# CentreForHydrology/WDPM

Hardware: AMD Instinct MI355X
Metric: cell-updates/sec on Add module, 16384x16384 DEM (higher is better)
Workload: dtype f64

## Files before the change

### wdpm_amd/csrc/wdpm_capi.hip

```cpp
#include <hip/hip_runtime.h>

#include <time.h>

#include <cmath>
#include <cstdarg>
#include <cstdio>
#include <cstdlib>
#include <cstring>
#include <atomic>
#include <vector>

#include "wdpm_ctx.h"

constexpr int kSparseChunkRows = 96;

static thread_local char g_err[512] = "";

int wdpm_fail(const char *fmt, ...) {
  va_list ap;
  va_start(ap, fmt);
  vsnprintf(g_err, sizeof g_err, fmt, ap);
  va_end(ap);
  return 1;
}
// ... 250 lines not shown
  x->w_negative = false;
  x->w_odd = true;
  x->launches = 0;
  x->ms = 0.0;
  x->steady_launches = 0;
  x->steady_ms = 0.0;
  x->timing = false; x->xch_count = 0; x->xch_ms = 0.0;
  x->comm = nullptr;
  x->leak = false;
  x->d_dem = x->d_w[0] = x->d_w[1] = x->d_w[2] = nullptr;
  x->old = 2;
  for (int i = 0; i < 3; i++) { x->d_zero[i] = nullptr; x->zero_valid[i] = false; }
  x->tile_cap = x->tile_nstrips = x->tile_H = x->tile_nchunks = 0;
  x->d_active = nullptr; x->h_active = nullptr;
  x->tiles_launched = 0; x->sparse = false; x->stat_tiles = x->stat_active = 0;
  x->wide_tri_ok = false; x->blocks_unprobed = 0;
  memset(&x->bal, 0, sizeof x->bal);
  { const char *e = getenv("WDPM_TILES"); x->tiles_mode = e ? atoi(e) : 1; }
  x->flush_pending = false;
  x->d_md = nullptr; x->md_hint = x->md_valid = false; x->md_lo = x->md_hi = 0;
  x->drain_owed = false;
  x->flush_thres = -__builtin_inf();
  x->d_scal = nullptr; x->d_bits = nullptr; x->h_pin = nullptr; x->d_stat = nullptr; x->h_iter2_err = x->d_iter2_err = nullptr;
  x->d_dem32 = nullptr; x->code = DemCode{nullptr, 0.0, 1.0, 1.0, 0, nullptr, nullptr, 0}; x->dem32_encodable = false; x->dem_bounded = false;
  x->d_dem16 = nullptr; x->d_gbase = nullptr; x->dem16_encodable = false; x->dem16_wanted = true;
  x->graph_mode = -1; x->graph_launches = 0;
  x->d_sum_approx = nullptr; x->d_sum_i = nullptr; x->d_sum_k = nullptr; x->d_sum_flag = nullptr;
  x->own_stream = true;
  x->side = nullptr; x->ev_fork = nullptr; x->ev_join = nullptr; x->pending_join = false; x->ev_copy[0] = x->ev_copy[1] = nullptr;
  const size_t bytes = x->cells * sizeof(double);
  hipError_t e = hipStreamCreateWithFlags(&x->stream, hipStreamNonBlocking);
  int prio_least = 0, prio_greatest = 0;
  if (e == hipSuccess) e = hipDeviceGetStreamPriorityRange(&prio_least, &prio_greatest);
  if (e == hipSuccess) e = hipStreamCreateWithPriority(&x->side, hipStreamNonBlocking, prio_least);
  if (e == hipSuccess) e = hipEventCreateWithFlags(&x->ev_fork, hipEventDisableTiming);
  if (e == hipSuccess) e = hipEventCreateWithFlags(&x->ev_join, hipEventDisableTiming);
  if (e == hipSuccess) e = guarded_malloc(x, (void **)&x->d_dem, bytes + 192 * sizeof(double));
  if (e == hipSuccess) e = guarded_malloc(x, (void **)&x->d_w[0], bytes + 192 * sizeof(double));
  if (e == hipSuccess) e = guarded_malloc(x, (void **)&x->d_w[1], bytes + 192 * sizeof(double));
  if (e == hipSuccess) e = guarded_malloc(x, (void **)&x->d_w[2], bytes + 192 * sizeof(double));
  if (e == hipSuccess) e = guarded_malloc(x, (void **)&x->d_dem32, x->cells * sizeof(int) + 64);
  if (e == hipSuccess) e = guarded_malloc(x, (void **)&x->d_dem16, x->cells * sizeof(unsigned short) + 64);
  if (e == hipSuccess) e = guarded_malloc(x, (void **)&x->d_gbase, (size_t)x->g.rows * ((x->g.ncp + kDemGroup - 1) / kDemGroup) * sizeof(int) + 64);
  if (e == hipSuccess) e = hipMalloc(&x->d_scal, 2 * sizeof(double));
  if (e == hipSuccess) e = hipMalloc(&x->d_bits, 2 * sizeof(unsigned long long));
  if (e == hipSuccess) e = hipMalloc(&x->d_md, sizeof(unsigned long long));
  if (e == hipSuccess) {
// ... 123 lines not shown
  q.flags = launch_flags(x);
  q.leave_cus = leave_cus;
  q.codes32 = x->code.q != nullptr;
  q.codes16 = x->code.h != nullptr;
  q.force_codes = x->code.force;
  q.tiles_offered = tiles != nullptr;
  q.tile_capacity = tiles && tiles->zout ? tiles->capacity : 0;
  q.wide_tri_ok = tiles && tiles->wide_tri_ok;
  q.balance_mode = balanced ? x->bal.mode : 0;
  q.balance_capacity = x->bal.capacity;
  return q;
}

static void drop_graphs(wdpm_ctx *x) {
  if (x->graphs.empty()) return;
  (void)hipStreamSynchronize(x->stream);
  for (auto &ge : x->graphs) (void)hipGraphExecDestroy(ge.exec);
  x->graphs.clear();
}

static int encode_dem(wdpm_ctx *x) {
  drop_graphs(x);
  x->dem32_encodable = false; x->dem16_encodable = false; x->dem_bounded = false; x->dem16_wanted = true;
  x->code = DemCode{nullptr, 0.0, 1.0, 1.0, 0, nullptr, nullptr, 0};
  HIP_TRY(wdpm_launch_dem_min(x->d_dem, x->cells, x->d_bits, x->stream));
  HIP_TRY(hipMemcpyAsync(x->h_pin, x->d_bits, 2 * sizeof(double), hipMemcpyDeviceToHost, x->stream));
  if (wdpm_stream_sync(x, x->stream)) return 1;
  unsigned long long key, amax;
  memcpy(&key, x->h_pin, sizeof key);
  memcpy(&amax, x->h_pin + 1, sizeof amax);
  x->dem_bounded = amax < 0x41d0000000000000ull;
  const char *env = getenv("WDPM_DEM32");
  if (env && atoi(env) == 0) return 0;
  if (key == ~0ull) return 0;
  const double vmin = wdpm_dem_key_to_double(key);
  static const double p10[7] = {1.0, 1e1, 1e2, 1e3, 1e4, 1e5, 1e6};
  for (int e = 0; e <= 6; e++) {
    const double D = p10[e], rD = 1.0 / D, k0 = rint(vmin * D);
    if (!(fabs(k0) < 4.0e15)) break;
    HIP_TRY(wdpm_launch_dem_encode(x->d_dem, x->cells, k0, D, rD, x->d_dem32, x->d_bits, x->stream));
    HIP_TRY(hipMemcpyAsync(x->h_pin, x->d_bits, sizeof(double), hipMemcpyDeviceToHost, x->stream));
    if (wdpm_stream_sync(x, x->stream)) return 1;
    unsigned long long bad;
    memcpy(&bad, x->h_pin, sizeof bad);
    if (!bad) {
      x->dem32_encodable = true;
      x->code = DemCode{x->d_dem32, k0, D, rD, (env && atoi(env) == 2) ? 1 : 0, nullptr, nullptr, 0};
      break;
    }
  }
  const char *env16 = getenv("WDPM_DEM16");
  if (x->dem32_encodable && !(env16 && atoi(env16) == 0)) {
    const int ngroups = (x->g.ncp + kDemGroup - 1) / kDemGroup;
    HIP_TRY(wdpm_launch_dem16_encode(x->d_dem32, x->g.rows, x->g.ncp, ngroups, x->d_dem16, x->d_gbase, x->d_bits, x->stream));
    HIP_TRY(hipMemcpyAsync(x->h_pin, x->d_bits, sizeof(double), hipMemcpyDeviceToHost, x->stream));
    if (wdpm_stream_sync(x, x->stream)) return 1;
    unsigned long long bad;
    memcpy(&bad, x->h_pin, sizeof bad);
    if (!bad) {
      x->dem16_encodable = true;
      x->code.h = x->d_dem16;
      x->code.gb = x->d_gbase;
      x->code.ngroups = ngroups;
    }
  }
  return 0;
}

int wdpm_upload(wdpm_ctx *x, const double *bigdem, const double *bigwater) {
  if (!bigdem || !bigwater) return fail("wdpm_upload: null array");
  if (bind(x)) return 1;
  const size_t bytes = x->cells * sizeof(double);
  if (ensure_fresh_slot(x)) return 1;
  HIP_TRY(hipMemcpyAsync(x->d_dem, bigdem, bytes, hipMemcpyHostToDevice, x->stream));
  HIP_TRY(hipMemcpyAsync(x->d_w[x->cur], bigwater, bytes, hipMemcpyHostToDevice, x->stream));
  HIP_TRY(wdpm_launch_mark_nodata(x->d_dem, x->cells, x->g.miss, x->stream));
  x->signed_zero_safe = x->w_negative = x->w_odd = false;
// ... 739 lines not shown
```

### wdpm_amd/csrc/wdpm_fused.hip

```cpp
#include "wdpm_kernels.h"
#include "wdpm_ledger.h"
#include "wdpm_stencil.h"

#include <atomic>
#include <cstring>
#include <mutex>
#include <type_traits>

namespace {


#define WDPM_INF (__builtin_inf())

__device__ __forceinline__ double lane_next(const double v) {
  int lo = __double2loint(v), hi = __double2hiint(v);
  lo = __builtin_amdgcn_update_dpp(0, lo, 0x130, 0xF, 0xF, true);
  hi = __builtin_amdgcn_update_dpp(0, hi, 0x130, 0xF, 0xF, true);
  return __hiloint2double(hi, lo);
}

__device__ __forceinline__ double lane_prev(const double v, const double keep) {
  int lo = __double2loint(v), hi = __double2hiint(v);
  lo = __builtin_amdgcn_update_dpp(__double2loint(keep), lo, 0x138, 0xF, 0xF, false);
  hi = __builtin_amdgcn_update_dpp(__double2hiint(keep), hi, 0x138, 0xF, 0xF, false);
// ... 149 lines not shown
                       D[a][2], da0, da1, D[b][2], db0, db1, D[c][2], dc0, dc1,
                       rd0, rd1, rd2, cdr[2], cdr[3], cdr[4], ds);
  W[a][0] = lane_prev(wa0, W[a][0]);  W[a][1] = lane_prev(wa1, W[a][1]);
  W[b][0] = lane_prev(wb0, W[b][0]);  W[b][1] = lane_prev(wb1, W[b][1]);
  W[c][0] = lane_prev(wc0, W[c][0]);  W[c][1] = lane_prev(wc1, W[c][1]);
}

template <int MODULE, bool SZ_SAFE, int NSTAGES = 3, int PLAIN = 0>
__device__ __forceinline__ void three_stages(double (&W)[7][3], const double (&D)[7][3], const int rbase,
                                             const int drain_row, const bool (&cdr)[5], DrainState &ds) {
  if (MODULE == 2 && drain_row >= rbase && drain_row <= rbase + 6) {
    stage_impl<MODULE, SZ_SAFE, 4, true>(W, D, rbase + 4, drain_row, cdr, ds);
    if (NSTAGES >= 2) stage_impl<MODULE, SZ_SAFE, 2, true>(W, D, rbase + 2, drain_row, cdr, ds);
    if (NSTAGES >= 3) stage_impl<MODULE, SZ_SAFE, 0, true>(W, D, rbase + 0, drain_row, cdr, ds);
  } else {
    stage_impl<MODULE, SZ_SAFE, 4, false, PLAIN>(W, D, rbase + 4, drain_row, cdr, ds);
    if (NSTAGES >= 2) stage_impl<MODULE, SZ_SAFE, 2, false, PLAIN>(W, D, rbase + 2, drain_row, cdr, ds);
    if (NSTAGES >= 3) stage_impl<MODULE, SZ_SAFE, 0, false, PLAIN>(W, D, rbase + 0, drain_row, cdr, ds);
  }
}

#ifdef WDPM_WAVE_TIMES
static __device__ unsigned long long g_wave_times[4 * 8192];
#define WDPM_RSTAMP(k) do { __builtin_amdgcn_sched_barrier(0); __builtin_amdgcn_s_waitcnt(0); rst[k] = wall_clock64(); __builtin_amdgcn_s_waitcnt(0); __builtin_amdgcn_sched_barrier(0); } while (0)
#else
#define WDPM_RSTAMP(k) do { } while (0)
#endif
#ifndef WDPM_FUSED_MIN_WAVES
#define WDPM_FUSED_MIN_WAVES 2
#endif
#ifndef WDPM_FUSED_CODES_WAVES
#define WDPM_FUSED_CODES_WAVES 2
#endif

typedef int wdpm_i3 __attribute__((ext_vector_type(3)));
struct Prefetched {
  double NW[3][3], ND[3][3];
  wdpm_i3 qi[3];
  int qh[3][3];
  int gbv[3];
};

template <int MODULE, bool SZ_SAFE, int DEM32, bool MD>
constexpr int fused_built_for() {
  return (MODULE == 2 && SZ_SAFE) ? 1 : (MODULE != 2 && DEM32 != 0 && !MD && !SZ_SAFE) ? WDPM_FUSED_CODES_WAVES : WDPM_FUSED_MIN_WAVES;
}

constexpr int kIter2Polls = 1 << 21;

template <int DEM32>
__device__ __forceinline__ void iter2_march(const double *__restrict__ win, double *__restrict__ wout, const DemCode &code, const SlabGeom &g,
                                            const int H, const int out_last, const int no_clamp, const BalanceArgs &bal, const Iter2Args &i2,
                                            const int vb, const int wave, const int lane, const int share, const int xcc_phys,
                                            double *const stage_lds) {
  extern __shared__ double i2_ring[];
  __shared__ int hand[8];
  if (threadIdx.x < 8) hand[threadIdx.x] = 0;
  __syncthreads();
  if (vb >= i2.ngroups * i2.nchunks) return;
#ifdef WDPM_WAVE_TIMES
  const unsigned long long wt0 = wall_clock64();
#endif
  const int grp = vb % i2.ngroups, chunk = vb / i2.ngroups;
  const bool producer = wave < 4;
  const int j = wave & 3;
  const int c0 = kGroupOut * grp + kStripOut * j;
  int A = H * chunk, A_next = A + H;
  if (bal.table) {
    A = bal.table[chunk * i2.ngroups + grp];
    A_next = bal.table[(chunk + 1) * i2.ngroups + grp];
    A = A < 0 ? 0 : (A > g.rows ? g.rows : A);
// ... 17 lines not shown
  int scol[3];
  bool store_any;
  {
    const int lo = j == 0 ? (grp == 0 ? 0 : kGroupHaloL) : kHaloL;
    int hi = kStripIn - 1 - (j == 3 ? kGroupHaloR : kHaloR);
    if (hi > g.ncp - 1 - c0) hi = g.ncp - 1 - c0;
    store_any = hi >= lo;
#pragma unroll
    for (int k = 0; k < 3; k++) {
      int c = lo + 64 * k + lane < hi ? lo + 64 * k + lane : hi;
      c = store_any ? c : 0;
      scol[k] = c;
      soff[k] = 8u * (unsigned)c;
    }
  }
  int dcol[3];
#pragma unroll
  for (int jj = 0; jj < 3; jj++) {
    const int cs = 3 * lane + jj;
    const bool own = cs >= (j == 0 ? 0 : kHaloL) && cs <= (j == 3 ? kStripIn - 1 : kStripIn - 1 - kHaloR);
    dcol[jj] = own ? kStripOut * j + cs : kGroupIn + jj;
  }
  const int rcol = kStripOut * j + 3 * lane;
  volatile int *const hand_v = hand;
  const int nb_lo = j > 0 ? j - 1 : 0, nb_hi = j < 3 ? j + 1 : 3;
  bool broken = false;
  auto await = [&](const int base, const int need) -> int {
    int m = 0, polls = 0;
    for (;;) {
      const int a = hand_v[base + nb_lo], b = hand_v[base + j], c = hand_v[base + nb_hi];
      m = a < b ? a : b;
      m = m < c ? m : c;
      m = __builtin_amdgcn_readfirstlane(m);
      if (m >= need || broken) break;
      if (++polls > kIter2Polls) {
        broken = true;
        if (lane == 0) *i2.err = 1u;
        break;
      }
      __builtin_amdgcn_s_sleep(2);
    }
    asm volatile("" ::: "memory");
    return m;
  };
  const size_t pitch = (size_t)g.ncp;
  char *const dump = reinterpret_cast<char *>(wout + (size_t)g.rows * pitch);
  const bool edge = (As + 3 * (nsteps + 1) > g.rows);
  double W[7][3], D[7][3];
#pragma unroll
  for (int k = 0; k < 7; k++)
#pragma unroll
    for (int jj = 0; jj < 3; jj++) { W[k][jj] = 0.0; D[k][jj] = WDPM_INF; }
  bool cdr[5];
#pragma unroll
  for (int k = 0; k < 5; k++) cdr[k] = false;
  DrainState ds;
  ds.td = 0.0;
  ds.hit = false;

  auto march = [&](auto edge_tag, auto role_tag) {
    constexpr bool EDGE = decltype(edge_tag)::value;
    constexpr bool PRODUCER = decltype(role_tag)::value;
    const int voff0 = 8 * (colb < g.ncp ? colb : g.ncp - 1);
    const int qoff0 = voff0 / 2, hoff0 = voff0 / 4, goff0 = 4 * ((voff0 / 8) / kDemGroup);
    auto prefetch = [&](Prefetched &P, const int r0) {
#pragma unroll
      for (int i = 0; i < 3; i++) {
// ... 46 lines not shown
      hand_v[4 + j] = t + 1;
    };
    double staged[3][3];
    auto read_staged = [&]() {
#pragma unroll
      for (int i = 0; i < 3; i++)
#pragma unroll
        for (int k = 0; k < 3; k++) staged[i][k] = stage_lds[i * kStripIn + scol[k]];
    };
    auto write_staged = [&](const int rb) {
#pragma unroll
      for (int i = 0; i < 3; i++) {
        const int r = rb + i;
        const bool row_ok = r >= or_lo && r <= or_hi && store_any;
        char *const orow = row_ok ? reinterpret_cast<char *>(wout + (size_t)r * pitch + c0) : dump;
#pragma unroll
        for (int k = 0; k < 3; k++) asm volatile("global_store_dwordx2 %0, %1, %2" : : "v"(soff[k]), "v"(staged[i][k]), "s"(orow) : "memory");
      }
      __builtin_amdgcn_wave_barrier();
    };

    auto step = [&](const int n, Prefetched &P, auto nstages_tag) {
      constexpr int NSTAGES = decltype(nstages_tag)::value;
      if (!PRODUCER) read_staged();
#pragma unroll
      for (int i = 0; i < 3; i++)
#pragma unroll
        for (int jj = 0; jj < 3; jj++) {
          W[4 + i][jj] = P.NW[i][jj];
          if (DEM32 == 2) D[4 + i][jj] = dem16_decode_nan(P.qh[i][jj], P.gbv[i], code.k0, code.D, code.rD);
          else D[4 + i][jj] = dem32_decode_nan(P.qi[i][jj], code.k0, code.D, code.rD);
        }
      if (EDGE) {
#pragma unroll
        for (int i = 0; i < 3; i++) {
          const bool row_ok = As + 3 * n + i < g.rows;
#pragma unroll
          for (int jj = 0; jj < 3; jj++) {
            const bool ok = row_ok & (colb + jj < g.ncp);
            W[4 + i][jj] = ok ? W[4 + i][jj] : 0.0;
            D[4 + i][jj] = ok ? D[4 + i][jj] : WDPM_INF;
          }
        }
      }
      {
        auto hi = [](const double v) { return (unsigned)__double2hiint(v); };
        auto max3 = [](const unsigned a, const unsigned b, const unsigned c) { const unsigned m = a > b ? a : b; return m > c ? m : c; };
        unsigned hm = max3(hi(W[4][0]), hi(W[4][1]), hi(W[4][2]));
        hm = max3(hm, hi(W[5][0]), hi(W[5][1]));
        hm = max3(hm, hi(W[5][2]), hi(W[6][0]));
        hm = max3(hm, hi(W[6][1]), hi(W[6][2]));
        deep = (deep & 8) | ((deep & 3) << 1) | (__ballot(hm > 0x40080000u) != 0 ? 1 : 0);
      }
      if (!PRODUCER) take(P, n + 1);
      prefetch(P, As + 3 * (n + 1));
      if (!PRODUCER) write_staged(A + 3 * (n - 1) - 4);

      const int rbase = As + 3 * n - 4;
      if (deep) three_stages<0, false, NSTAGES, 1>(W, D, rbase, g.dr, cdr, ds);
      else three_stages<0, false, NSTAGES, 1 | 2>(W, D, rbase, g.dr, cdr, ds);

      if (PRODUCER) {
        const int rr0 = 3 * n - 4 - sh;
        const int taken = await(4, n - sh / 3 - R / 3);
        if (i2.prio) {
          const int ahead = n - lag - taken;
          if (ahead <= 1) __builtin_amdgcn_s_setprio(3);
          else if (ahead >= R / 3 - 1) __builtin_amdgcn_s_setprio(0);
          else __builtin_amdgcn_s_setprio(1);
        }
#pragma unroll
        for (int i = 0; i < 3; i++) {
          double *const row = i2_ring + (size_t)(rr0 + i >= 0 ? put_slot : R) * kRingPitch;
          if (rr0 + i >= 0) put_slot = put_slot + 1 >= R ? 0 : put_slot + 1;
#pragma unroll
          for (int jj = 0; jj < 3; jj++) row[dcol[jj]] = W[i][jj];
        }
        asm volatile("" ::: "memory");
        hand_v[j] = n + 1;
      } else {
#pragma unroll
        for (int i = 0; i < 3; i++)
#pragma unroll
// ... 25 lines not shown
  };
  if (producer) {
    if (edge) march(std::true_type{}, std::true_type{});
    else march(std::false_type{}, std::true_type{});
  } else {
    if (edge) march(std::true_type{}, std::false_type{});
    else march(std::false_type{}, std::false_type{});
  }
  if (bal.acc && lane == 0) {
    const int x = chunk == i2.nchunks - 1 ? 8 : chunk == 0 ? 9 : (bal.rot ? xcc_phys : (int)(blockIdx.x & 7));
    if (!bal.rot || share == xcc_phys) {
      atomicAdd(bal.acc + x, wall_clock64() - bal_t0);
      atomicAdd(bal.acc + kBalClasses + x, 1ull);
    }
  }
#ifdef WDPM_WAVE_TIMES
  const int item = vb * 8 + wave;
  if (lane == 0 && item < 8192) {
    __builtin_amdgcn_s_waitcnt(0);
    g_wave_times[4 * item] = wt0;
    g_wave_times[4 * item + 1] = wall_clock64();
    g_wave_times[4 * item + 2] = __builtin_amdgcn_s_getreg((31 << 11) | 4) | ((unsigned long long)__builtin_amdgcn_s_getreg((3 << 11) | 20) << 32);
    g_wave_times[4 * item + 3] = ((unsigned long long)(4 * grp + j + (producer ? 0 : 0x4000)) << 48) | ((unsigned long long)(nsteps & 0xffff) << 32) | (unsigned)chunk;
  }
#endif
}

template <int MODULE, bool SZ_SAFE, int DEM32, bool FLUSH = false, bool MD = false, bool PLAIN = false>
__global__ void __launch_bounds__((fused_built_for<MODULE, SZ_SAFE, DEM32, MD>() >= 2 ? 512 : 256), (fused_built_for<MODULE, SZ_SAFE, DEM32, MD>()))
fused_iteration_kernel(const double *__restrict__ win, double *__restrict__ wout,
                       const double *__restrict__ dem, const DemCode code, const SlabGeom g, const int nstrips,
                       const int nitems, const int H, const int A0, const int out_last,
                       double *__restrict__ totaldrain, const double thres, const int drain_owed,
                       const TileFlags tf, const MaxDiffArgs md, const int prio, const int no_clamp, const BalanceArgs bal, const Iter2Args i2) {
  const int lane = threadIdx.x & 63;
  const int xcc_phys = (int)(__builtin_amdgcn_s_getreg((3 << 11) | 20) & 7);
  int rot_prev = 0;
  if (bal.rot) {
    rot_prev = __builtin_amdgcn_readfirstlane((int)(bal.rot[bal.parity] & 7));
    if (blockIdx.x == 0 && threadIdx.x == 0) bal.rot[bal.parity ^ 1] = (unsigned long long)xcc_phys;
  }
  const int share = (int)((blockIdx.x + (unsigned)rot_prev) % 8);
#ifdef WDPM_XCD_REVERSE
  const int vb = (7 - share) * (gridDim.x / 8) + blockIdx.x / 8;
#elif defined(WDPM_ORDER_REVERSE)
  const int vb = share * (gridDim.x / 8) + (gridDim.x / 8 - 1 - blockIdx.x / 8);
// ... 209 lines not shown
        char *const orow = row_ok ? reinterpret_cast<char *>(wout + (size_t)((WDPM_ABLATE_HBM & 2) ? r % 48 : r) * pitch + c0) : dump;
#else
        char *const orow = row_ok ? reinterpret_cast<char *>(wout + (size_t)r * pitch + c0) : dump;
#endif
#pragma unroll
        for (int k = 0; k < 3; k++) asm volatile("global_store_dwordx2 %0, %1, %2" : : "v"(soff[k]), "v"(staged[i][k]), "s"(orow) : "memory");
      }
      __builtin_amdgcn_wave_barrier();
    };

    auto step = [&](const int n, Prefetched &P, auto nstages_tag) {
      constexpr int NSTAGES = decltype(nstages_tag)::value;
      int partner_at = 0;
      if (use_prio) {
        *my_progress = n;
        partner_at = *partner_progress;
      }
      read_staged();
#pragma unroll
      for (int i = 0; i < 3; i++)
#pragma unroll
        for (int j = 0; j < 3; j++) {
          W[4 + i][j] = FLUSH && P.NW[i][j] < thres ? 0.0 : P.NW[i][j];
          if (DEM32 == 2) D[4 + i][j] = dem16_decode_nan(P.qh[i][j], P.gbv[i], code.k0, code.D, code.rD);
          else if (DEM32) D[4 + i][j] = dem32_decode_nan(P.qi[i][j], code.k0, code.D, code.rD);
          else D[4 + i][j] = P.ND[i][j];
        }
      if (MODULE == 2 && owed_here && A + 3 * n + 2 >= g.dr - 1 && A + 3 * n <= g.dr + 1) {
#pragma unroll
        for (int i = 0; i < 3; i++) {
          const bool owed_row = A + 3 * n + i >= g.dr - 1 && A + 3 * n + i <= g.dr + 1;
#pragma unroll
          for (int j = 0; j < 3; j++) W[4 + i][j] = owed_row && owed_col[j] ? 0.0 : W[4 + i][j];
        }
      }
      if (EDGE) {
#pragma unroll
        for (int i = 0; i < 3; i++) {
          const bool row_ok = A + 3 * n + i < g.rows;
#pragma unroll
          for (int j = 0; j < 3; j++) {
            const bool ok = row_ok & (colb + j < g.ncp);
            W[4 + i][j] = ok ? W[4 + i][j] : 0.0;
            D[4 + i][j] = ok ? D[4 + i][j] : WDPM_INF;
          }
        }
      }
      if constexpr (!SZ_SAFE) {
// ... 411 lines not shown
  if (or_hi > out_last) or_hi = out_last;
  const int R0 = A + 3 * wave;
  const int colb = c0 + 3 * lane;
  const size_t pitch = (size_t)g.ncp;
#ifdef WDPM_WAVE_TIMES
  unsigned long long rst[8];
  rst[0] = wall_clock64();
#endif
  const bool rprio = (store_plain & 2) != 0;
  if (rprio) __builtin_amdgcn_s_setprio(3);
  unsigned voff[3];
#pragma unroll
  for (int j = 0; j < 3; j++) voff[j] = 8u * (unsigned)(colb + j < g.ncp ? colb + j : g.ncp - 1);
  double W[7][3], D[7][3];
  constexpr bool LDSDEM = NW == 8 || MODULE == 2;
#pragma unroll
  for (int i = 0; i < (LDSDEM ? 3 : 5); i++) {
    const int rc = R0 + i < g.rows ? R0 + i : g.rows - 1;
    const char *bw = reinterpret_cast<const char *>(win + (size_t)rc * pitch);
    const char *bd = reinterpret_cast<const char *>(dem + (size_t)rc * pitch);
    const char *bq = reinterpret_cast<const char *>(code.q + (size_t)rc * pitch);
#pragma unroll
    for (int j = 0; j < 3; j++) {
      if (DEM32) D[i][j] = dem32_decode_nan(*reinterpret_cast<const int *>(bq + voff[j] / 2), code.k0, code.D, code.rD);
      else D[i][j] = *reinterpret_cast<const double *>(bd + voff[j]);
      W[i][j] = i < 3 ? *reinterpret_cast<const double *>(bw + voff[j]) : 0.0;
    }
  }
#pragma unroll
  for (int i = (LDSDEM ? 3 : 5); i < 7; i++)
#pragma unroll
    for (int j = 0; j < 3; j++) { W[i][j] = 0.0; D[i][j] = WDPM_INF; }

  DrainState ds;
  ds.td = 0.0;
  ds.hit = false;
  bool owner = false;
  int wo[3] = {-1, -1, -1};
  bool cdr[5];
#pragma unroll
  for (int j = 0; j < 5; j++) cdr[j] = MODULE == 2 && colb + j == g.dc;
  if (MODULE == 2) {
    const bool outlet_inside = g.dr >= 1 && g.dr <= g.rows - 2 && g.dc >= 1 && g.dc <= g.ncp - 2;
    const bool col_here = g.dc >= c0 && g.dc <= c0 + kStripIn + 1;
#pragma unroll
    for (int st = 0; st < 3; st++) {
      const int rel = g.dr - A - st;
// ... 375 lines not shown
    e = tiles_hand_over(b.tiles, p, b.stream, &tf);
    if (e != hipSuccess) return e;
  }
  const MaxDiffArgs mda = p.fold_md ? *b.md : MaxDiffArgs{nullptr, 0.0, 0, 0, nullptr};
  if (p.fold_md) tf = TileFlags{nullptr, nullptr, 0, nullptr, p.nchunks};
  if (p.fold_md && b.tiles) b.tiles->maintained = 0;
  const BalanceArgs ba = p.balance ? balance_step(b.bal, q, p, b.stream) : BalanceArgs{nullptr, nullptr, nullptr, 0};
  if (p.iter2 && !b.iter2_err) return hipErrorInvalidValue;
  const Iter2Args i2{p.iter2, p.nstrips, p.nchunks, p.ring_rows, p.iter2_prio, b.iter2_err};
  wdpm_ledger_count(*kMarchingTable[at].slot, p.ledger_sw);
  hipLaunchKernelGGL(kMarchingTable[at].fn, dim3(p.grid), dim3(p.block), p.lds, b.stream, b.w_in, b.w_out, b.dem, *b.code, q.g, p.nstrips, p.nitems,
                     p.H, q.A0, q.out_last, b.totaldrain, b.thres, q.module == 2 ? b.drain_owed : 0, tf, mda, p.prio, p.no_clamp, ba, i2);
  return hipGetLastError();
}

#endif

#ifdef WDPM_WAVE_TIMES
#if !defined(WDPM_TU) || WDPM_TU == 1
extern "C" int wdpm_debug_wave_times(unsigned long long *out, int nwaves) {
  if (hipDeviceSynchronize() != hipSuccess) return 1;
  return hipMemcpyFromSymbol(out, HIP_SYMBOL(g_wave_times), (size_t)nwaves * 32) != hipSuccess;
}
#endif
#if !defined(WDPM_TU) || WDPM_TU == 2
extern "C" int wdpm_debug_relay_times(unsigned long long *out, int nwaves) {
  if (hipDeviceSynchronize() != hipSuccess) return 1;
  return hipMemcpyFromSymbol(out, HIP_SYMBOL(g_wave_times), (size_t)nwaves * 32) != hipSuccess;
}
#endif
#endif
```

### wdpm_amd/csrc/wdpm_kernels.h

```cpp
#ifndef WDPM_KERNELS_H
#define WDPM_KERNELS_H

#include <hip/hip_runtime.h>
#include <stdint.h>

#include "wdpm_dispatch.h"

struct DemCode {
  const int *q;
  double k0;
  double D, rD;
  int force;
  const unsigned short *h;
  const int *gb;
  int ngroups;
};
constexpr int kDemGroup = 48;
hipError_t wdpm_launch_dem_min(const double *dem, size_t cells, unsigned long long *key, hipStream_t s);
double wdpm_dem_key_to_double(unsigned long long key);
hipError_t wdpm_launch_dem_encode(const double *dem, size_t cells, double k0, double D, double rD, int *q,
                                  unsigned long long *bad, hipStream_t s);

hipError_t wdpm_launch_dem16_encode(const int *q, int rows, int ncp, int ngroups, unsigned short *h, int *gb,
                                    unsigned long long *bad, hipStream_t s);

constexpr int kSeqSumChunk = 65536;
hipError_t wdpm_launch_seqsum_a(const double *w, const double *dem, size_t n, double *approx, unsigned *dirty,
                                hipStream_t s);
hipError_t wdpm_launch_seqsum_b(const double *w, const double *dem, size_t n, const int *kexp, long long *isum,
                                unsigned *tie, hipStream_t s);

struct TileFlags {
  const unsigned char *zin;
  unsigned char *zout;
  int zout_known;
  unsigned *active;
  int nchunks;
};
struct TilePlan {
  const unsigned char *zin;
  unsigned char *zout;
  int zin_valid, zout_valid;
  unsigned *active;
  int capacity;
  int nstrips, H, nchunks;
  int maintained;
// ... 78 lines not shown
```

### wdpm_amd/csrc/wdpm_kernels.hip

```cpp
#include "wdpm_kernels.h"
#include "wdpm_ledger.h"
#include "wdpm_stencil.h"

__device__ __forceinline__ bool cell_valid(const double dem) { return dem < __builtin_inf(); }

__global__ void __launch_bounds__(256)
mark_nodata_kernel(double *__restrict__ dem, size_t cells, double miss) {
  const size_t stride = (size_t)gridDim.x * blockDim.x;
  for (size_t i = (size_t)blockIdx.x * blockDim.x + threadIdx.x; i < cells; i += stride) {
    const double d = dem[i];
    if (!(d > miss)) dem[i] = __builtin_inf();
  }
}

hipError_t wdpm_launch_mark_nodata(double *dem, size_t cells, double miss, hipStream_t s) {
  size_t blocks = (cells + 255) / 256;
  if (blocks > 4096) blocks = 4096;
  WDPM_LEDGER(0, mark_nodata_kernel);
  hipLaunchKernelGGL(mark_nodata_kernel, dim3((unsigned)blocks), dim3(256), 0, s, dem, cells, miss);
  return hipGetLastError();
}

template <int MODULE>
__global__ void __launch_bounds__(256)
// ... 135 lines not shown
    }
  }
#pragma unroll
  for (int off = 32; off >= 1; off >>= 1) {
    const unsigned long long o = __shfl_xor(m, off, 64), oa = __shfl_xor(a, off, 64);
    m = o < m ? o : m;
    a = oa > a ? oa : a;
  }
  if ((threadIdx.x & 63) == 0 && m != ~0ull) { atomicMin(key, m); atomicMax(key + 1, a); }
}

hipError_t wdpm_launch_dem_min(const double *dem, size_t cells, unsigned long long *key, hipStream_t s) {
  hipError_t e = hipMemsetAsync(key, 0xff, sizeof(unsigned long long), s);
  if (e == hipSuccess) e = hipMemsetAsync(key + 1, 0, sizeof(unsigned long long), s);
  if (e != hipSuccess || cells == 0) return e;
  size_t blocks = (cells + 255) / 256;
  if (blocks > 2048) blocks = 2048;
  WDPM_LEDGER(0, dem_min_kernel);
  hipLaunchKernelGGL(dem_min_kernel, dim3((unsigned)blocks), dim3(256), 0, s, dem, cells, key);
  return hipGetLastError();
}

__global__ void __launch_bounds__(256)
dem_encode_kernel(const double *__restrict__ dem, size_t n, double k0, double D, double rD, int *__restrict__ q,
                  unsigned long long *bad) {
  const size_t stride = (size_t)gridDim.x * blockDim.x;
  bool miss = false;
  for (size_t i = (size_t)blockIdx.x * blockDim.x + threadIdx.x; i < n; i += stride) {
    const double v = dem[i];
    int code = (int)0x80000000;
    if (cell_valid(v)) {
      const double kk = rint(v * D) - k0;
      const bool fits = fabs(kk) < 2147483647.0;
      code = fits ? (int)kk : 0;
      const bool same = __double_as_longlong(dem32_decode(code, k0, D, rD)) == __double_as_longlong(v);
      miss |= !(fits && same);
    }
    q[i] = code;
  }
  if (__ballot(miss) && (threadIdx.x & 63) == 0) atomicOr(bad, 1ull);
}

hipError_t wdpm_launch_dem_encode(const double *dem, size_t cells, double k0, double D, double rD, int *q,
                                  unsigned long long *bad, hipStream_t s) {
  hipError_t e = hipMemsetAsync(bad, 0, sizeof(unsigned long long), s);
  if (e != hipSuccess || cells == 0) return e;
  size_t blocks = (cells + 255) / 256;
  if (blocks > 4096) blocks = 4096;
  WDPM_LEDGER(0, dem_encode_kernel);
  hipLaunchKernelGGL(dem_encode_kernel, dim3((unsigned)blocks), dim3(256), 0, s, dem, cells, k0, D, rD, q, bad);
  return hipGetLastError();
}

__global__ void __launch_bounds__(256)
dem16_encode_kernel(const int *__restrict__ q, int rows, int ncp, int ngroups, unsigned short *__restrict__ h,
                    int *__restrict__ gb, unsigned long long *bad) {
  const size_t total = (size_t)rows * ngroups, stride = (size_t)gridDim.x * blockDim.x;
  bool miss = false;
  for (size_t i = (size_t)blockIdx.x * blockDim.x + threadIdx.x; i < total; i += stride) {
    const int r = (int)(i / ngroups), g = (int)(i % ngroups);
    const int c0 = g * kDemGroup, c1 = c0 + kDemGroup < ncp ? c0 + kDemGroup : ncp;
    const int *row = q + (size_t)r * ncp;
    long long lo = 0x7fffffffLL, hi = -0x80000000LL;
    for (int c = c0; c < c1; c++) {
      const int v = row[c];
      if (v != (int)0x80000000) { lo = v < lo ? v : lo; hi = v > hi ? v : hi; }
    }
    if (hi < lo) lo = hi = 0;
    miss |= hi - lo > 65534;
    gb[i] = (int)lo;
    for (int c = c0; c < c1; c++) {
      const int v = row[c];
      h[(size_t)r * ncp + c] = v == (int)0x80000000 ? (unsigned short)0xFFFF : (unsigned short)((long long)v - lo);
    }
  }
  if (__ballot(miss) && (threadIdx.x & 63) == 0) atomicOr(bad, 1ull);
}

hipError_t wdpm_launch_dem16_encode(const int *q, int rows, int ncp, int ngroups, unsigned short *h, int *gb,
                                    unsigned long long *bad, hipStream_t s) {
  hipError_t e = hipMemsetAsync(bad, 0, sizeof(unsigned long long), s);
  if (e != hipSuccess || rows <= 0) return e;
  size_t blocks = ((size_t)rows * ngroups + 255) / 256;
  if (blocks > 65536) blocks = 65536;
  WDPM_LEDGER(0, dem16_encode_kernel);
  hipLaunchKernelGGL(dem16_encode_kernel, dim3((unsigned)blocks), dim3(256), 0, s, q, rows, ncp, ngroups, h, gb, bad);
  return hipGetLastError();
}

__global__ void __launch_bounds__(256)
seqsum_a_kernel(const double *__restrict__ w, const double *__restrict__ dem, size_t n, double *approx,
                unsigned *dirty) {
  __shared__ double part[4];
  const size_t lo = (size_t)blockIdx.x * kSeqSumChunk, hi = lo + kSeqSumChunk < n ? lo + kSeqSumChunk : n;
  double s = 0.0;
  bool bad = false;
  for (size_t i = lo + threadIdx.x; i < hi; i += 256)
    if (cell_valid(dem[i])) {
      const double v = w[i];
      bad |= !(v >= 0.0) | (v == __builtin_inf());
      s += v;
    }
#pragma unroll
  for (int off = 32; off >= 1; off >>= 1) s += __shfl_xor(s, off, 64);
  if ((threadIdx.x & 63) == 0) part[threadIdx.x >> 6] = s;
  const bool any_bad = __syncthreads_or(bad);
  if (threadIdx.x == 0) {
    approx[blockIdx.x] = (part[0] + part[1]) + (part[2] + part[3]);
    dirty[blockIdx.x] = any_bad ? 1u : 0u;
// ... 269 lines not shown
```

### wdpm_amd/csrc/wdpm_stencil.h

```cpp
#ifndef WDPM_STENCIL_H
#define WDPM_STENCIL_H

#include <hip/hip_runtime.h>

__device__ __forceinline__ double dem32_decode(const int q, const double k0, const double D, const double rD) {
  const double n = (double)q + k0;
  const double q0 = n * rD;
  const double r = __builtin_fma(-q0, D, n);
  const double v = __builtin_fma(r, rD, q0);
  return q == (int)0x80000000 ? __builtin_inf() : v;
}

__device__ __forceinline__ double dem32_decode_nan(const int q, const double k0, const double D, const double rD) {
  const double n = (double)q + k0;
  const double q0 = n * rD;
  const double r = __builtin_fma(-q0, D, n);
  const double v = __builtin_fma(r, rD, q0);
  const int hi = q == (int)0x80000000 ? 0x7ff80000 : __double2hiint(v);
  return __hiloint2double(hi, __double2loint(v));
}

__device__ __forceinline__ double dem16_decode_nan(const int h, const int gb, const double k0, const double D, const double rD) {
  const double n = (double)(gb + h) + k0;
  const double q0 = n * rD;
  const double r = __builtin_fma(-q0, D, n);
  const double v = __builtin_fma(r, rD, q0);
  const int hi = h == 0xFFFF ? 0x7ff80000 : __double2hiint(v);
  return __hiloint2double(hi, __double2loint(v));
}

__host__ __device__ constexpr int nb_dr(int k) { return (k < 3) ? -1 : (k < 5 ? 0 : 1); }
__host__ __device__ constexpr int nb_dc(int k) { return (k < 3) ? k - 1 : (k == 3 ? -1 : (k == 4 ? 1 : k - 6)); }

__device__ __forceinline__ double vmin_f64(const double a, const double b) {
  double r;
  asm("v_min_f64 %0, %1, %2" : "=v"(r) : "v"(a), "v"(b));
  return r;
}
__device__ __forceinline__ double vmax_f64(const double a, const double b) {
  double r;
  asm("v_max_f64 %0, %1, %2" : "=v"(r) : "v"(a), "v"(b));
  return r;
}

__device__ __forceinline__ void flow_add(const double dem_c, double &w_c, const double dem_n, double &w_n,
                                         const bool gate = true) {
  const double en = dem_n + w_n;
  const double ht = (dem_c + w_c) - en;
  const bool go = gate & (ht > 0);
// ... 56 lines not shown
```

Baseline: 258.7 billion.

## Use two-term reciprocal DEM decode, retire idle iter2 waves, defer take

```diff
diff --git a/wdpm_amd/csrc/wdpm_capi.hip b/wdpm_amd/csrc/wdpm_capi.hip
--- a/wdpm_amd/csrc/wdpm_capi.hip
+++ b/wdpm_amd/csrc/wdpm_capi.hip
@@ -296,7 +296,7 @@
   x->drain_owed = false;
   x->flush_thres = -__builtin_inf();
   x->d_scal = nullptr; x->d_bits = nullptr; x->h_pin = nullptr; x->d_stat = nullptr; x->h_iter2_err = x->d_iter2_err = nullptr;
-  x->d_dem32 = nullptr; x->code = DemCode{nullptr, 0.0, 1.0, 1.0, 0, nullptr, nullptr, 0}; x->dem32_encodable = false; x->dem_bounded = false;
+  x->d_dem32 = nullptr; x->code = DemCode{nullptr, 0.0, 1.0, 1.0, 0.0, 0, nullptr, nullptr, 0}; x->dem32_encodable = false; x->dem_bounded = false;
   x->d_dem16 = nullptr; x->d_gbase = nullptr; x->dem16_encodable = false; x->dem16_wanted = true;
   x->graph_mode = -1; x->graph_launches = 0;
   x->d_sum_approx = nullptr; x->d_sum_i = nullptr; x->d_sum_k = nullptr; x->d_sum_flag = nullptr;
@@ -466,7 +466,7 @@
 static int encode_dem(wdpm_ctx *x) {
   drop_graphs(x);
   x->dem32_encodable = false; x->dem16_encodable = false; x->dem_bounded = false; x->dem16_wanted = true;
-  x->code = DemCode{nullptr, 0.0, 1.0, 1.0, 0, nullptr, nullptr, 0};
+  x->code = DemCode{nullptr, 0.0, 1.0, 1.0, 0.0, 0, nullptr, nullptr, 0};
   HIP_TRY(wdpm_launch_dem_min(x->d_dem, x->cells, x->d_bits, x->stream));
   HIP_TRY(hipMemcpyAsync(x->h_pin, x->d_bits, 2 * sizeof(double), hipMemcpyDeviceToHost, x->stream));
   if (wdpm_stream_sync(x, x->stream)) return 1;
@@ -481,22 +481,23 @@
   static const double p10[7] = {1.0, 1e1, 1e2, 1e3, 1e4, 1e5, 1e6};
   for (int e = 0; e <= 6; e++) {
     const double D = p10[e], rD = 1.0 / D, k0 = rint(vmin * D);
+    const double rDlo = fma(-rD, D, 1.0) / D;
     if (!(fabs(k0) < 4.0e15)) break;
-    HIP_TRY(wdpm_launch_dem_encode(x->d_dem, x->cells, k0, D, rD, x->d_dem32, x->d_bits, x->stream));
+    HIP_TRY(wdpm_launch_dem_encode(x->d_dem, x->cells, k0, D, rD, rDlo, x->d_dem32, x->d_bits, x->stream));
     HIP_TRY(hipMemcpyAsync(x->h_pin, x->d_bits, sizeof(double), hipMemcpyDeviceToHost, x->stream));
     if (wdpm_stream_sync(x, x->stream)) return 1;
     unsigned long long bad;
     memcpy(&bad, x->h_pin, sizeof bad);
     if (!bad) {
       x->dem32_encodable = true;
-      x->code = DemCode{x->d_dem32, k0, D, rD, (env && atoi(env) == 2) ? 1 : 0, nullptr, nullptr, 0};
+      x->code = DemCode{x->d_dem32, k0, D, rD, rDlo, (env && atoi(env) == 2) ? 1 : 0, nullptr, nullptr, 0};
       break;
     }
   }
   const char *env16 = getenv("WDPM_DEM16");
   if (x->dem32_encodable && !(env16 && atoi(env16) == 0)) {
     const int ngroups = (x->g.ncp + kDemGroup - 1) / kDemGroup;
-    HIP_TRY(wdpm_launch_dem16_encode(x->d_dem32, x->g.rows, x->g.ncp, ngroups, x->d_dem16, x->d_gbase, x->d_bits, x->stream));
+    HIP_TRY(wdpm_launch_dem16_encode(x->code, x->g.rows, x->g.ncp, ngroups, x->d_dem16, x->d_gbase, x->d_bits, x->stream));
     HIP_TRY(hipMemcpyAsync(x->h_pin, x->d_bits, sizeof(double), hipMemcpyDeviceToHost, x->stream));
     if (wdpm_stream_sync(x, x->stream)) return 1;
     unsigned long long bad;
diff --git a/wdpm_amd/csrc/wdpm_fused.hip b/wdpm_amd/csrc/wdpm_fused.hip
--- a/wdpm_amd/csrc/wdpm_fused.hip
+++ b/wdpm_amd/csrc/wdpm_fused.hip
@@ -195,6 +195,7 @@
 
 #ifdef WDPM_WAVE_TIMES
 static __device__ unsigned long long g_wave_times[4 * 8192];
+static __device__ unsigned long long g_wave_waits[4 * 8192];
 #define WDPM_RSTAMP(k) do { __builtin_amdgcn_sched_barrier(0); __builtin_amdgcn_s_waitcnt(0); rst[k] = wall_clock64(); __builtin_amdgcn_s_waitcnt(0); __builtin_amdgcn_sched_barrier(0); } while (0)
 #else
 #define WDPM_RSTAMP(k) do { } while (0)
@@ -220,6 +221,7 @@
 }
 
 constexpr int kIter2Polls = 1 << 21;
+constexpr int kIter2Retired = 1 << 30;
 
 template <int DEM32>
 __device__ __forceinline__ void iter2_march(const double *__restrict__ win, double *__restrict__ wout, const DemCode &code, const SlabGeom &g,
@@ -283,11 +285,22 @@
     dcol[jj] = own ? kStripOut * j + cs : kGroupIn + jj;
   }
   const int rcol = kStripOut * j + 3 * lane;
+#ifdef WDPM_ITER2_FLAT_HAND
   volatile int *const hand_v = hand;
+#else
+  volatile __attribute__((address_space(3))) int *const hand_v = (volatile __attribute__((address_space(3))) int *)hand;
+#endif
   const int nb_lo = j > 0 ? j - 1 : 0, nb_hi = j < 3 ? j + 1 : 3;
   bool broken = false;
+#ifdef WDPM_WAVE_TIMES
+  unsigned wt_polls0 = 0, wt_polls1 = 0, wt_polls2 = 0, wt_ticks0 = 0, wt_ticks1 = 0, wt_ticks2 = 0, wt_waits = 0;
+  int wt_phase = 0;
+#endif
   auto await = [&](const int base, const int need) -> int {
     int m = 0, polls = 0;
+#ifdef WDPM_WAVE_TIMES
+    unsigned long long wt_a = 0;
+#endif
     for (;;) {
       const int a = hand_v[base + nb_lo], b = hand_v[base + j], c = hand_v[base + nb_hi];
       m = a < b ? a : b;
@@ -299,11 +312,38 @@
         if (lane == 0) *i2.err = 1u;
         break;
       }
+#ifdef WDPM_WAVE_TIMES
+      if (polls == 1) wt_a = wall_clock64();
+#endif
       __builtin_amdgcn_s_sleep(2);
     }
+#ifdef WDPM_WAVE_TIMES
+    if (polls) {
+      const unsigned dt = (unsigned)(wall_clock64() - wt_a);
+      wt_waits++;
+      if (wt_phase == 0) { wt_polls0 += polls; wt_ticks0 += dt; }
+      else if (wt_phase == 1) { wt_polls1 += polls; wt_ticks1 += dt; }
+      else { wt_polls2 += polls; wt_ticks2 += dt; }
+    }
+#endif
     asm volatile("" ::: "memory");
     return m;
   };
+#ifdef WDPM_ITER2_NO_RETIRE
+  const bool retire = false;
+#else
+  const bool retire = producer ? c0 + (j == 0 ? 0 : kHaloL) >= g.ncp : !store_any;
+#endif
+  if (retire) {
+    if (producer) {
+      for (int r = 0; r < R; r++)
+#pragma unroll
+        for (int jj = 0; jj < 3; jj++) i2_ring[(size_t)r * kRingPitch + dcol[jj]] = 0.0;
+      asm volatile("" ::: "memory");
+    }
+    hand_v[wave] = kIter2Retired;
+    return;
+  }
   const size_t pitch = (size_t)g.ncp;
   char *const dump = reinterpret_cast<char *>(wout + (size_t)g.rows * pitch);
   const bool edge = (As + 3 * (nsteps + 1) > g.rows);
@@ -396,14 +436,17 @@
 
     auto step = [&](const int n, Prefetched &P, auto nstages_tag) {
       constexpr int NSTAGES = decltype(nstages_tag)::value;
+#ifdef WDPM_WAVE_TIMES
+      wt_phase = n < 4 ? 0 : (n >= nsteps - 4 ? 2 : 1);
+#endif
       if (!PRODUCER) read_staged();
 #pragma unroll
       for (int i = 0; i < 3; i++)
 #pragma unroll
         for (int jj = 0; jj < 3; jj++) {
           W[4 + i][jj] = P.NW[i][jj];
-          if (DEM32 == 2) D[4 + i][jj] = dem16_decode_nan(P.qh[i][jj], P.gbv[i], code.k0, code.D, code.rD);
-          else D[4 + i][jj] = dem32_decode_nan(P.qi[i][jj], code.k0, code.D, code.rD);
+          if (DEM32 == 2) D[4 + i][jj] = dem16_decode_nan(P.qh[i][jj], P.gbv[i], code.k0, code.D, code.rD, code.rDlo);
+          else D[4 + i][jj] = dem32_decode_nan(P.qi[i][jj], code.k0, code.D, code.rD, code.rDlo);
         }
       if (EDGE) {
 #pragma unroll
@@ -426,13 +469,18 @@
         hm = max3(hm, hi(W[6][1]), hi(W[6][2]));
         deep = (deep & 8) | ((deep & 3) << 1) | (__ballot(hm > 0x40080000u) != 0 ? 1 : 0);
       }
+#ifdef WDPM_ITER2_EARLY_TAKE
       if (!PRODUCER) take(P, n + 1);
+#endif
       prefetch(P, As + 3 * (n + 1));
       if (!PRODUCER) write_staged(A + 3 * (n - 1) - 4);
 
       const int rbase = As + 3 * n - 4;
       if (deep) three_stages<0, false, NSTAGES, 1>(W, D, rbase, g.dr, cdr, ds);
       else three_stages<0, false, NSTAGES, 1 | 2>(W, D, rbase, g.dr, cdr, ds);
+#ifndef WDPM_ITER2_EARLY_TAKE
+      if (!PRODUCER) take(P, n + 1);
+#endif
 
       if (PRODUCER) {
         const int rr0 = 3 * n - 4 - sh;
@@ -504,6 +552,10 @@
     g_wave_times[4 * item + 1] = wall_clock64();
     g_wave_times[4 * item + 2] = __builtin_amdgcn_s_getreg((31 << 11) | 4) | ((unsigned long long)__builtin_amdgcn_s_getreg((3 << 11) | 20) << 32);
     g_wave_times[4 * item + 3] = ((unsigned long long)(4 * grp + j + (producer ? 0 : 0x4000)) << 48) | ((unsigned long long)(nsteps & 0xffff) << 32) | (unsigned)chunk;
+    g_wave_waits[4 * item] = wt_polls0 | ((unsigned long long)wt_polls1 << 32);
+    g_wave_waits[4 * item + 1] = wt_polls2 | ((unsigned long long)wt_waits << 32);
+    g_wave_waits[4 * item + 2] = wt_ticks0 | ((unsigned long long)wt_ticks1 << 32);
+    g_wave_waits[4 * item + 3] = wt_ticks2;
   }
 #endif
 }
@@ -759,8 +811,8 @@
 #pragma unroll
         for (int j = 0; j < 3; j++) {
           W[4 + i][j] = FLUSH && P.NW[i][j] < thres ? 0.0 : P.NW[i][j];
-          if (DEM32 == 2) D[4 + i][j] = dem16_decode_nan(P.qh[i][j], P.gbv[i], code.k0, code.D, code.rD);
-          else if (DEM32) D[4 + i][j] = dem32_decode_nan(P.qi[i][j], code.k0, code.D, code.rD);
+          if (DEM32 == 2) D[4 + i][j] = dem16_decode_nan(P.qh[i][j], P.gbv[i], code.k0, code.D, code.rD, code.rDlo);
+          else if (DEM32) D[4 + i][j] = dem32_decode_nan(P.qi[i][j], code.k0, code.D, code.rD, code.rDlo);
           else D[4 + i][j] = P.ND[i][j];
         }
       if (MODULE == 2 && owed_here && A + 3 * n + 2 >= g.dr - 1 && A + 3 * n <= g.dr + 1) {
@@ -1218,7 +1270,7 @@
     const char *bq = reinterpret_cast<const char *>(code.q + (size_t)rc * pitch);
 #pragma unroll
     for (int j = 0; j < 3; j++) {
-      if (DEM32) D[i][j] = dem32_decode_nan(*reinterpret_cast<const int *>(bq + voff[j] / 2), code.k0, code.D, code.rD);
+      if (DEM32) D[i][j] = dem32_decode_nan(*reinterpret_cast<const int *>(bq + voff[j] / 2), code.k0, code.D, code.rD, code.rDlo);
       else D[i][j] = *reinterpret_cast<const double *>(bd + voff[j]);
       W[i][j] = i < 3 ? *reinterpret_cast<const double *>(bw + voff[j]) : 0.0;
     }
@@ -1640,6 +1692,10 @@
   if (hipDeviceSynchronize() != hipSuccess) return 1;
   return hipMemcpyFromSymbol(out, HIP_SYMBOL(g_wave_times), (size_t)nwaves * 32) != hipSuccess;
 }
+extern "C" int wdpm_debug_wave_waits(unsigned long long *out, int nwaves) {
+  if (hipDeviceSynchronize() != hipSuccess) return 1;
+  return hipMemcpyFromSymbol(out, HIP_SYMBOL(g_wave_waits), (size_t)nwaves * 32) != hipSuccess;
+}
 #endif
 #if !defined(WDPM_TU) || WDPM_TU == 2
 extern "C" int wdpm_debug_relay_times(unsigned long long *out, int nwaves) {
diff --git a/wdpm_amd/csrc/wdpm_kernels.h b/wdpm_amd/csrc/wdpm_kernels.h
--- a/wdpm_amd/csrc/wdpm_kernels.h
+++ b/wdpm_amd/csrc/wdpm_kernels.h
@@ -10,6 +10,7 @@
   const int *q;
   double k0;
   double D, rD;
+  double rDlo;
   int force;
   const unsigned short *h;
   const int *gb;
@@ -18,10 +19,10 @@
 constexpr int kDemGroup = 48;
 hipError_t wdpm_launch_dem_min(const double *dem, size_t cells, unsigned long long *key, hipStream_t s);
 double wdpm_dem_key_to_double(unsigned long long key);
-hipError_t wdpm_launch_dem_encode(const double *dem, size_t cells, double k0, double D, double rD, int *q,
+hipError_t wdpm_launch_dem_encode(const double *dem, size_t cells, double k0, double D, double rD, double rDlo, int *q,
                                   unsigned long long *bad, hipStream_t s);
 
-hipError_t wdpm_launch_dem16_encode(const int *q, int rows, int ncp, int ngroups, unsigned short *h, int *gb,
+hipError_t wdpm_launch_dem16_encode(const DemCode &code, int rows, int ncp, int ngroups, unsigned short *h, int *gb,
                                     unsigned long long *bad, hipStream_t s);
 
 constexpr int kSeqSumChunk = 65536;
diff --git a/wdpm_amd/csrc/wdpm_kernels.hip b/wdpm_amd/csrc/wdpm_kernels.hip
--- a/wdpm_amd/csrc/wdpm_kernels.hip
+++ b/wdpm_amd/csrc/wdpm_kernels.hip
@@ -181,7 +181,7 @@
 }
 
 __global__ void __launch_bounds__(256)
-dem_encode_kernel(const double *__restrict__ dem, size_t n, double k0, double D, double rD, int *__restrict__ q,
+dem_encode_kernel(const double *__restrict__ dem, size_t n, double k0, double D, double rD, double rDlo, int *__restrict__ q,
                   unsigned long long *bad) {
   const size_t stride = (size_t)gridDim.x * blockDim.x;
   bool miss = false;
@@ -192,7 +192,7 @@
       const double kk = rint(v * D) - k0;
       const bool fits = fabs(kk) < 2147483647.0;
       code = fits ? (int)kk : 0;
-      const bool same = __double_as_longlong(dem32_decode(code, k0, D, rD)) == __double_as_longlong(v);
+      const bool same = __double_as_longlong(dem32_decode(code, k0, D, rD, rDlo)) == __double_as_longlong(v);
       miss |= !(fits && same);
     }
     q[i] = code;
@@ -200,20 +200,20 @@
   if (__ballot(miss) && (threadIdx.x & 63) == 0) atomicOr(bad, 1ull);
 }
 
-hipError_t wdpm_launch_dem_encode(const double *dem, size_t cells, double k0, double D, double rD, int *q,
+hipError_t wdpm_launch_dem_encode(const double *dem, size_t cells, double k0, double D, double rD, double rDlo, int *q,
                                   unsigned long long *bad, hipStream_t s) {
   hipError_t e = hipMemsetAsync(bad, 0, sizeof(unsigned long long), s);
   if (e != hipSuccess || cells == 0) return e;
   size_t blocks = (cells + 255) / 256;
   if (blocks > 4096) blocks = 4096;
   WDPM_LEDGER(0, dem_encode_kernel);
-  hipLaunchKernelGGL(dem_encode_kernel, dim3((unsigned)blocks), dim3(256), 0, s, dem, cells, k0, D, rD, q, bad);
-  return hipGetLastError();
-}
-
-__global__ void __launch_bounds__(256)
-dem16_encode_kernel(const int *__restrict__ q, int rows, int ncp, int ngroups, unsigned short *__restrict__ h,
-                    int *__restrict__ gb, unsigned long long *bad) {
+  hipLaunchKernelGGL(dem_encode_kernel, dim3((unsigned)blocks), dim3(256), 0, s, dem, cells, k0, D, rD, rDlo, q, bad);
+  return hipGetLastError();
+}
+
+__global__ void __launch_bounds__(256)
+dem16_encode_kernel(const int *__restrict__ q, int rows, int ncp, int ngroups, double k0, double D, double rD, double rDlo,
+                    unsigned short *__restrict__ h, int *__restrict__ gb, unsigned long long *bad) {
   const size_t total = (size_t)rows * ngroups, stride = (size_t)gridDim.x * blockDim.x;
   bool miss = false;
   for (size_t i = (size_t)blockIdx.x * blockDim.x + threadIdx.x; i < total; i += stride) {
@@ -230,20 +230,24 @@
     gb[i] = (int)lo;
     for (int c = c0; c < c1; c++) {
       const int v = row[c];
-      h[(size_t)r * ncp + c] = v == (int)0x80000000 ? (unsigned short)0xFFFF : (unsigned short)((long long)v - lo);
+      const unsigned short hv = v == (int)0x80000000 ? (unsigned short)0xFFFF : (unsigned short)((long long)v - lo);
+      h[(size_t)r * ncp + c] = hv;
+      if (v != (int)0x80000000)
+        miss |= __double_as_longlong(dem16_decode_nan((int)hv, (int)lo, k0, D, rD, rDlo)) != __double_as_longlong(dem32_decode_nan(v, k0, D, rD, rDlo));
     }
   }
   if (__ballot(miss) && (threadIdx.x & 63) == 0) atomicOr(bad, 1ull);
 }
 
-hipError_t wdpm_launch_dem16_encode(const int *q, int rows, int ncp, int ngroups, unsigned short *h, int *gb,
+hipError_t wdpm_launch_dem16_encode(const DemCode &code, int rows, int ncp, int ngroups, unsigned short *h, int *gb,
                                     unsigned long long *bad, hipStream_t s) {
   hipError_t e = hipMemsetAsync(bad, 0, sizeof(unsigned long long), s);
   if (e != hipSuccess || rows <= 0) return e;
   size_t blocks = ((size_t)rows * ngroups + 255) / 256;
   if (blocks > 65536) blocks = 65536;
   WDPM_LEDGER(0, dem16_encode_kernel);
-  hipLaunchKernelGGL(dem16_encode_kernel, dim3((unsigned)blocks), dim3(256), 0, s, q, rows, ncp, ngroups, h, gb, bad);
+  hipLaunchKernelGGL(dem16_encode_kernel, dim3((unsigned)blocks), dim3(256), 0, s, code.q, rows, ncp, ngroups, code.k0, code.D, code.rD,
+                     code.rDlo, h, gb, bad);
   return hipGetLastError();
 }
 
diff --git a/wdpm_amd/csrc/wdpm_stencil.h b/wdpm_amd/csrc/wdpm_stencil.h
--- a/wdpm_amd/csrc/wdpm_stencil.h
+++ b/wdpm_amd/csrc/wdpm_stencil.h
@@ -3,28 +3,34 @@
 
 #include <hip/hip_runtime.h>
 
-__device__ __forceinline__ double dem32_decode(const int q, const double k0, const double D, const double rD) {
-  const double n = (double)q + k0;
+__device__ __forceinline__ double dem_quotient(const double n, const double D, const double rD, const double rDlo) {
+#ifdef WDPM_DECODE_NEWTON
   const double q0 = n * rD;
   const double r = __builtin_fma(-q0, D, n);
-  const double v = __builtin_fma(r, rD, q0);
+  return __builtin_fma(r, rD, q0);
+#else
+  return __builtin_fma(n, rD, n * rDlo);
+#endif
+}
+
+__device__ __forceinline__ double dem32_decode(const int q, const double k0, const double D, const double rD, const double rDlo) {
+  const double v = dem_quotient((double)q + k0, D, rD, rDlo);
   return q == (int)0x80000000 ? __builtin_inf() : v;
 }
 
-__device__ __forceinline__ double dem32_decode_nan(const int q, const double k0, const double D, const double rD) {
-  const double n = (double)q + k0;
-  const double q0 = n * rD;
-  const double r = __builtin_fma(-q0, D, n);
-  const double v = __builtin_fma(r, rD, q0);
+__device__ __forceinline__ double dem32_decode_nan(const int q, const double k0, const double D, const double rD, const double rDlo) {
+  const double v = dem_quotient((double)q + k0, D, rD, rDlo);
   const int hi = q == (int)0x80000000 ? 0x7ff80000 : __double2hiint(v);
   return __hiloint2double(hi, __double2loint(v));
 }
 
-__device__ __forceinline__ double dem16_decode_nan(const int h, const int gb, const double k0, const double D, const double rD) {
+__device__ __forceinline__ double dem16_decode_nan(const int h, const int gb, const double k0, const double D, const double rD, const double rDlo) {
+#ifdef WDPM_DECODE_NEWTON
   const double n = (double)(gb + h) + k0;
-  const double q0 = n * rD;
-  const double r = __builtin_fma(-q0, D, n);
-  const double v = __builtin_fma(r, rD, q0);
+#else
+  const double n = ((double)gb + k0) + (double)(unsigned)h;
+#endif
+  const double v = dem_quotient(n, D, rD, rDlo);
   const int hi = h == 0xFFFF ? 0x7ff80000 : __double2hiint(v);
   return __hiloint2double(hi, __double2loint(v));
 }
```

Result: faster. 265.9 billion (median of 6 runs) (+2.8%).
